# dayae1204/WeCLIP-ViT-CoMer

Measured on AMD Instinct MI355X. Metric: images/sec (train fwd+bwd) ViT-B/16 512x512 VOC, higher is better.
Workload: dtype f16 MFMA operands / f32 accumulate, f32 residual+softmax+LN, PAR f32 arithmetic on 16-bit fixed-point affinities (precision=fast); 1 GPU; WeCLIP VOC full train step (the reference's model: frozen CLIP ViT-B/16 + adapters + decoder + GradCAM/affinity/PAR pseudo-labels), batch 16/GPU at 512x512, K=2 classes/image (BASELINE configs[2] without the ViT-CoMer inserts, for which the reference has no code); global_batch=16, parallelism=dp1

## Files before the change

include/weclip_hip.h:

```cpp
#ifndef WECLIP_HIP_H
#define WECLIP_HIP_H
#include <stdint.h>
#ifdef __cplusplus
extern "C" {
#endif

int wc_version(void);
const char* wc_last_error(void);
int wc_device_count(void);
int wc_device_arch(int dev, char* buf, int buflen);

void wc_prof_enable(int stride);
void wc_prof_tag(const char* tag);
int wc_prof_report(char* buf, int cap);

int wc_par_affinity(const float* img, float* aff, int B, int H, int W,
                    const int* h_dilations, int n_dil, void* stream);
int wc_par_iterate(const float* aff, const float* masks_in, float* masks_out, int B, int C,
                   int H, int W, const int* h_dilations, int n_dil, void* stream);
int wc_par_forward(const float* img, const float* masks, float* out, float* tmp, float* aff_ws,
                   int B, int C, int H, int W, const int* h_dilations, int n_dil, int num_iter,
                   int group, void* stream);
int wc_par_forward_h(const float* img, const float* masks, float* out, float* tmp, float* aff_ws,
                   int B, int C, int H, int W, const int* h_dilations, int n_dil, int num_iter,
// ... 35 lines not shown
int wc_gemm_f16_grouped(const void* A0, const void* A1, const void* A2, const void* W0, const void* W1,
                        const void* W2, int nseg, int M, int N, int K, long lda, long ldw, int batch,
                        long sA, long sW, long sC, const float* bias, const float* resid, long ldr, long sR,
                        float* C32, void* C16, void* C16lo, long ldc, int act, int round16, float scale,
                        int scale_cols, float* P32, const float* aux, const int* rowmap, int rpg,
                        long ldaux, const void* auxh, const float* cscale, long sCS, int zdiv, long sA2, long sW2,
                        long sC2, long sB2, long sX2, void* stream);

int wc_gemm_row_supported(int M, int N, int K);
int wc_gemm_row_f16(const void* A, long lda, const void* W, long ldw, int M, int N, int K, const float* bias,
                    const float* cscale, int act, const float* aux, const void* auxh, long ldaux, const float* resid, long ldr,
                    float* C32, void* C16, float* P32, long ldc, long ldc16, const float* ln_g0, const float* ln_b0, void* ln_o0,
                    const float* ln_g1, const float* ln_b1, void* ln_o1, float eps, void* stream);

int wc_gemm_row_f16_grouped(const void* A, long lda, const void* W, long ldw, int M, int N, int K, const float* bias, int act,
                            const void* auxh, long ldaux, float* C32, void* C16, long ldc, long ldc16, int groups, long gA,
                            long gW, long gB, long gC, long gX, void* stream);

int wc_gemm_plan(int M, int N, int K, int nseg, int batch);
int wc_gemm_log_report(char* buf, int cap);
int wc_sum_slices(const float* part, float* out, int nslices, long n, float alpha, void* stream);

int wc_sum_slices_wb(const float* part, float* out_w, float* out_b, int nslices, int rows, int cols,
                     float alpha, void* stream);
int wc_sum_slices_wb_grouped(const float* part, float* out_w, float* out_b, int nslices, int rows, int cols,
                             float alpha, int groups, long gW, long gB, void* stream);
int wc_sum_slices_wb_multi(const int64_t* jobs, int count, void* stream);

int wc_gemm_km_f16(const void* dY, long lda, const void* X, long ldx, const void* zeros, int M, int N, int K,
                   int x_rpg, int x_gs, int x_off, int mslice, int bias, float* part, void* stream);
int wc_gemm_km_f16_grouped(const void* dY, long lda, const void* X, long ldx, const void* zeros, int M, int N, int K,
                           int x_rpg, int x_gs, int x_off, int mslice, int bias, float* part, int groups, long gA,
                           long gX, void* stream);
int wc_split_f16(const float* x, void* hi, void* lo, long n, void* stream);

int wc_convert_weights(const int64_t* table, int count, int blocks_per_tensor, void* stream);

int wc_adamw_multi(const int64_t* table, int count, double lr, double beta1, double beta2, double eps,
                   double weight_decay, double bias_correction1, double bias_correction2, int blocks_per_tensor,
                   void* stream);

int wc_layernorm(const float* x, long ldx, const float* w, const float* b, float eps, float* y32,
                 void* y16, void* y16lo, long rows, int D, void* stream);

int wc_attn_fwd(const void* qkv, void* out, float* out32, float* lse, int B, int L, int H, int DH,
                void* stream);
int wc_attn_mean(const void* qkv, const float* lse, float* mean, int B, int L, int H, int DH,
                 void* stream);

int wc_patchify(const float* img, void* hi, void* lo, int B, int H, int W, int P, void* stream);
int wc_cls_rows(float* x, const float* cls, const float* pos0, int B, int L, int E, void* stream);

int wc_cam_head(const float* x2, const float* lnw, const float* lnb, const float* proj,
                const float* text, const int* text_idx, const int* n_text, const int* pair_img,
                const int* pair_cls, float logit_scale, float* partial, float* probs, float* df,
                int B, int P, int L, int E, int Ed, int Tmax, void* stream);
int wc_lnpost_bwd(const float* df, const float* x2, const float* lnw, float gs, const int* pair_img,
                  float* d32, void* dhi, void* dlo, int P, int L, int E, void* stream);
int wc_ln2_bwd_add(const float* da2, const float* dx2, const float* x1, const float* lnw, float gs,
                   const int* pair_img, void* g16, int P, int L, int E, void* stream);
int wc_attn_bwd_colsum(const void* qkv, const void* dO, const float* o32, const float* lse,
                       const int* pair_img, float* delta, float* u, float* dS0, float* P0, float* c,
                       int P, int L, int H, int DH, void* stream);
int wc_rowvec_matmul(const float* c, const float* W, float* out, float* ws, int P, int N, int E, float scale,
                     void* stream);
int wc_cam_map(const float* a32, const float* w, const int* pair_img, float* cam, int P, int L, int E,
// ... 170 lines not shown
```

weclip-vit-comer_amd/build.py:

```python
import hashlib
import os
import subprocess
import sys
from concurrent.futures import ThreadPoolExecutor

HERE = os.path.dirname(os.path.abspath(__file__))
CSRC = os.path.join(HERE, "csrc")
OBJ = os.path.join(CSRC, "_build")
LIB = os.path.join(HERE, "libweclip_hip.so")
HIPCC = os.environ.get("HIPCC", "/opt/rocm/bin/hipcc")
FLAGS = ["--offload-arch=gfx950", "-O3", "-fPIC", "-std=c++17", "-ffp-contract=off",
         "-Wno-unused-result", "-I", CSRC] + os.environ.get("WECLIP_HIPCC_FLAGS", "").split()


NO_SCRATCH = ("gemm_row.hip",)


def _sources():
    return sorted(f for f in os.listdir(CSRC) if f.endswith(".hip"))


def _stamp(src):
    h = hashlib.sha1()
    h.update(" ".join("<csrc>" if f == CSRC else f for f in FLAGS).encode())
    for f in [src] + sorted(f for f in os.listdir(CSRC) if f.endswith(".h")):
        with open(os.path.join(CSRC, f), "rb") as fh:
            h.update(fh.read())
    return h.hexdigest()


def source_hash():
    h = hashlib.sha1()
    h.update(" ".join("<csrc>" if f == CSRC else f for f in FLAGS).encode())
    for f in sorted(f for f in os.listdir(CSRC) if f.endswith((".hip", ".h"))):
        with open(os.path.join(CSRC, f), "rb") as fh:
            h.update(f.encode())
            h.update(fh.read())
    return h.hexdigest()[:16]


def _compile(src):
    obj = os.path.join(OBJ, src[:-4] + ".o")
    stamp_file = obj + ".stamp"
    stamp = _stamp(src)
    if os.path.exists(obj) and os.path.exists(stamp_file) and open(stamp_file).read() == stamp:
        return obj, False
    cmd = [HIPCC] + FLAGS + ["-c", os.path.join(CSRC, src), "-o", obj]
    if src in NO_SCRATCH:
# ... 38 lines not shown
```

weclip-vit-comer_amd/comer_engine.py:

```python
import ctypes

import torch

from . import _lib as L
from . import config, ops
from .grad_sink import GradSink, handback, slices
from .ops import F16, F32, Split

GS = 4096.0
INV = 1.0 / GS


_WGRAD_WGS = 256


def _shape_array(shapes):
    return L.int_array([v for hw in shapes for v in hw])


class ComerEngine:
    def __init__(self, net):
        self.net = net
        self.wc = ops.WeightCache()
        self._ref = {}
        self.adapters = None
        self.row_gemm = True

    def params(self):
        net = self.net
        out = []
        for m, c in zip(net.mrfp, net.cti):
            out += [m.fc1.weight, m.fc1.bias, m.fc2.weight, m.fc2.bias, m.dw3.weight, m.dw3.bias, m.dw5.weight, m.dw5.bias]
            out += [c.nv_q.weight, c.nv_q.bias, c.nv_f.weight, c.nv_f.bias, c.gamma, c.nc_q.weight, c.nc_q.bias,
                    c.nc_f.weight, c.nc_f.bias, c.ffn_norm.weight, c.ffn_norm.bias,
                    c.ffn[0].weight, c.ffn[0].bias, c.ffn[2].weight, c.ffn[2].bias]
            for a in (c.to_v, c.to_c):
                out += [a.sampling_offsets.weight, a.sampling_offsets.bias, a.attention_weights.weight, a.attention_weights.bias,
                        a.value_proj.weight, a.value_proj.bias, a.output_proj.weight, a.output_proj.bias]
        out += [net.fuse.weight, net.fuse.bias]
        for a in (self.adapters or []):
            out += [a.proj.weight, a.proj.bias, a.proj_2.weight, a.proj_2.bias]
        return out

    def _mats(self):
        f = lambda t: t.detach() if (t.dtype == F32 and t.is_contiguous()) else t.detach().float().contiguous()
        out = []
        for i, (m, c) in enumerate(zip(self.net.mrfp, self.net.cti)):
            out += [(f"m{i}.fc1", f(m.fc1.weight)), (f"m{i}.fc2", f(m.fc2.weight)), (f"f{i}.0", f(c.ffn[0].weight)),
                    (f"f{i}.2", f(c.ffn[2].weight))]
            for tag, a in (("v", c.to_v), ("c", c.to_c)):
                out += [(f"{tag}{i}.vp", f(a.value_proj.weight)), (f"{tag}{i}.op", f(a.output_proj.weight)),
                        (f"{tag}{i}.ow", [f(a.sampling_offsets.weight), f(a.attention_weights.weight)])]
        out.append(("fuse", f(self.net.fuse.weight).flatten(1)))
# ... 264 lines not shown
                dvs[i] = self._ln_bwd(sink, dq1, s["v"], t.nv_q, dv1)
            df1 = torch.empty(Mc, C, device=dev, dtype=F16)
            self._mm(dval1_16, WT(f"v{i}.vp"), Mc, C, C, out16=df1)
            self._wgrad(sink, dval1_16, s["f1"], Mc, C, C, t.to_v.value_proj)
            if t.nc_q.eps == t.nv_f.eps and C <= 256:
                dc1, dc1_16 = self._ln_bwd2(sink, dq2, t.nc_q, df1, t.nv_f, s["c1"], dc2)
            else:
                dc1 = self._ln_bwd(sink, dq2, s["c1"], t.nc_q, dc2)
                dc1, dc1_16 = self._ln_bwd(sink, df1, s["c1"], t.nv_f, dc1, want16=True)
            dx2 = torch.empty(Mc, hid, device=dev, dtype=F16)
            self._mm(dc1_16, WT(f"m{i}.fc2"), Mc, hid, C, out16=dx2, act=7, aux=s["x2"], ldaux=hid, rpg=1)
            self._wgrad(sink, dc1_16, s["g16"], Mc, C, hid, m.fc2)
            dx1_16 = torch.empty(Mc, hid, device=dev, dtype=F16)
            dw3, db3, dw5, db5 = (sink.dest(q) for q in (m.dw3.weight, m.dw3.bias, m.dw5.weight, m.dw5.bias))
            npart = ctypes.c_long(0)
            lib.wc_mrfp_dwconv_parts(hs3, len(shapes), B, hid, ctypes.byref(npart))
            part = torch.empty(npart.value * hid * 26, device=dev, dtype=F32)
            lib.wc_mrfp_dwconv_bwd(L.ptr(dx2), 1, L.ptr(s["x1"]), L.ptr(self._b(m.dw3.weight).view(-1), F32),
                                   L.ptr(self._b(m.dw5.weight).view(-1), F32), None, L.ptr(dx1_16), L.ptr(dw3), L.ptr(db3), L.ptr(dw5),
                                   L.ptr(db5), L.ptr(part), INV, hs3, len(shapes), B, hid, L.stream())
            dc = torch.empty(Mc, C, device=dev, dtype=F32)
            self._mm(dx1_16, WT(f"m{i}.fc1"), Mc, C, hid, out32=dc, resid=dc1)
            self._wgrad(sink, dx1_16, s["c16"], Mc, hid, C, m.fc1)
            dc3 = dc
        return dc3, dvs

    def _ow_grads(self, sink, dow16, q16, M, n, ld, att):
        K = att.d_model
        outs = [(sink.dest(lin.weight), sink.dest(lin.bias)) for lin in (att.sampling_offsets, att.attention_weights)]
        sink.wgrad(dow16, q16, M, n, K, INV, outs, ns=slices(M, ops.wgrad_tiles(n, K), _WGRAD_WGS), lda=ld)

    def run_backward(self, ctx, dy):
        self._gamma_jobs = []
        with GradSink(self.net.direct_grads) as sink:
            dc0, dvs = self._backward(ctx, dy, sink)
        for t, G, gsum in self._gamma_jobs:
            op = t.to_v.output_proj
            dW, db, dg = (sink.dest(q) for q in (op.weight, op.bias, t.gamma))
            L.lib().wc_cti_gate_grads(L.ptr(G, F32), L.ptr(gsum, F32), L.ptr(self._b(t.gamma), F32), L.ptr(self._b(op.weight), F32),
                                      L.ptr(self._b(op.bias), F32), L.ptr(dW, F32), L.ptr(db, F32), L.ptr(dg, F32), G.shape[0], G.shape[1],
                                      L.stream())
        self._gamma_jobs = None
        B, S, C = ctx["B"], ctx["S"], ctx["C"]
        return (dc0 * INV).view(B, S, C), [d * INV if d is not None else None for d in dvs], sink.grads


class ComerFunction(torch.autograd.Function):

    @staticmethod
    def forward(ctx, engine, shapes, hw, c0, m0, m1, m2, m3, *params):
        y, c = engine.forward(c0, shapes, hw, [m0, m1, m2, m3])
        ctx.engine, ctx.c, ctx.map_shapes = engine, c, [m.shape for m in (m0, m1, m2, m3)]
        return y

    @staticmethod
    def backward(ctx, dy):
        eng = ctx.engine
        dc0, dvs, grads = eng.run_backward(ctx.c, dy.contiguous())
        ctx.c = None
        return (None, None, None, dc0) + tuple(d.view(s) for d, s in zip(dvs, ctx.map_shapes)) + handback(eng.params(), grads)


class ComerTokensFunction(torch.autograd.Function):

    @staticmethod
    def forward(ctx, engine, shapes, hw, Lq, c0, x0, x1, x2, x3, *params):
        y, c = engine.forward(c0, shapes, hw, None, x16=[x0, x1, x2, x3], Lq=Lq)
# ... 10 lines not shown
```

weclip-vit-comer_amd/csrc/gemm_km.hip:

```cpp
#include "gemm_common.h"
#include <cstring>
#include <stdlib.h>

struct KmArgs {
    const __half* A;
    const __half* X;
    const __half* zeros;
    int M, N, K;
    long lda, ldx;
    int x_rpg, x_gs, x_off;
    int mslice;
    int bias;
    int bias_edge;
    int gx;
    int tiles, ns, units;
    int xcd;
    long gA, gX, gP;
    GemmArgs e;
};

typedef short s16x4 __attribute__((__vector_size__(4 * sizeof(short))));
typedef short s16x8 __attribute__((__vector_size__(8 * sizeof(short))));

template <int NST, int HV>
__global__ __launch_bounds__(256 * HV, (HV == 1 && NST <= 5) ? 2 : 1) void gemm_km_kernel(KmArgs g) {
    extern __shared__ __attribute__((aligned(16))) char smem[];
    constexpr int ST = 32 * HV;
    constexpr int TILE = ST * 256;
    constexpr int NT_ = 256 * HV;
    const int tid = threadIdx.x, lane = tid & 63, wave = tid >> 6;
    const int half = HV == 2 ? wave >> 2 : 0, w4 = wave & 3;
    const int wr = w4 >> 1, wc = w4 & 1;
    int unit, tile;
    if (g.xcd) {
        const int chunk = blockIdx.x / (8 * g.tiles), within = blockIdx.x - chunk * (8 * g.tiles);
        unit = chunk * 8 + (within & 7);
        tile = within >> 3;
    } else {
        unit = blockIdx.x / g.tiles;
        tile = blockIdx.x - unit * g.tiles;
    }
    const int grp = unit / g.ns;
    const int z = unit - grp * g.ns;
    const int ty = tile / g.gx, tx = tile - ty * g.gx;
    const int n0 = ty * 128, k0 = tx * 128;
    const __half* Ag = g.A + (long)grp * g.gA;
    const __half* Xg = g.X + (long)grp * g.gX;
    const int mbeg = z * g.mslice;
    const int mend = (mbeg + g.mslice < g.M) ? mbeg + g.mslice : g.M;
    const int nt = (mend - mbeg + ST - 1) / ST;

    int rowi[2], acol[2], xcol[2], xg[2], xr[2];
    unsigned offA[2], offX[2];
    bool aok[2], xok[2];
#pragma unroll
    for (int i = 0; i < 2; ++i) {
        const int q = i * NT_ + tid;
        const int row = q >> 4, pc = q & 15;
        const int lc = pc ^ (((row & 3) << 2) | ((row >> 2) & 3));
        rowi[i] = row;
        acol[i] = n0 + lc * 8;
        xcol[i] = k0 + lc * 8;
        aok[i] = acol[i] + 8 <= g.lda && acol[i] < g.N;
        xok[i] = xcol[i] + 8 <= g.ldx && xcol[i] < g.K;
        const int m = mbeg + row;
        xg[i] = m / g.x_rpg;
        xr[i] = m - xg[i] * g.x_rpg;
        offA[i] = (unsigned)(((long)m * g.lda + (aok[i] ? acol[i] : 0)) * 2);
        offX[i] = (unsigned)((((long)xg[i] * g.x_gs + xr[i] + g.x_off) * g.ldx + (xok[i] ? xcol[i] : 0)) * 2);
    }
    const unsigned dA = (unsigned)(ST * g.lda * 2), dX = (unsigned)(ST * g.ldx * 2);
    const unsigned dXg = (unsigned)(((long)g.x_gs - g.x_rpg) * g.ldx * 2);
    typedef __attribute__((address_space(3))) void* lds_ptr;
    typedef const __attribute__((address_space(1))) void* gbl_ptr;
// ... 132 lines not shown
#pragma unroll
                for (int r = 0; r < 16; ++r) acc[i][j][r] += ex[((i * 2 + j) * 16 + r) * 64];
#pragma unroll
            for (int r = 0; r < 16; ++r) bacc[i][r] += ex[((4 + i) * 16 + r) * 64];
        }
    }
    if (edge_bias) {
        if ((lane & 31) == 0) {
            float* pb = g.e.C32 + (long)z * g.e.sC + (long)grp * g.gP + g.K;
#pragma unroll
            for (int mi = 0; mi < 2; ++mi)
#pragma unroll
                for (int r = 0; r < 16; ++r) {
                    const int row = n0 + wr * 64 + mi * 32 + (r & 3) + 8 * (r >> 2) + 4 * (lane >> 5);
                    if (row < g.N) pb[(long)row * g.e.ldc] = bacc[mi][r];
                }
        }
    } else if (own_bias) {
        const int ni = kb >> 5, cl = kb & 31;
        if ((lane & 31) == cl) {
#pragma unroll
            for (int mi = 0; mi < 2; ++mi)
#pragma unroll
                for (int r = 0; r < 16; ++r) {
                    if (ni == 0) acc[mi][0][r] = bacc[mi][r];
                    else acc[mi][1][r] = bacc[mi][r];
                }
        }
    }
    const float bv[2] = {0.f, 0.f}, sc[2] = {1.f, 1.f};
    gemm_epilogue<0>(g.e, acc, n0, k0, wr, wc, lane, z, smem + w4 * 8192, bv, sc, (long)z * g.e.sC + (long)grp * g.gP);
}

extern "C" int wc_gemm_km_f16_grouped(const void* dY, long lda, const void* X, long ldx, const void* zeros, int M, int N,
                                      int K, int x_rpg, int x_gs, int x_off, int mslice, int bias, float* part, int groups,
                                      long gA, long gX, void* stream) {
    WC_CHECK_ARG(dY && X && zeros && part && M > 0 && N > 0 && K > 0, "wc_gemm_km_f16: bad argument");
    WC_CHECK_ARG(groups >= 1 && groups <= 65535 && gA % 8 == 0 && gX % 8 == 0, "wc_gemm_km_f16_grouped: bad group strides");
    WC_CHECK_ARG(lda % 8 == 0 && ldx % 8 == 0 && lda >= N && ldx >= K && ((uintptr_t)dY | (uintptr_t)X | (uintptr_t)zeros) % 16 == 0,
                 "wc_gemm_km_f16: operand rows must be 16-byte aligned (lda, ldx %% 8 == 0)");
    WC_CHECK_ARG(mslice > 0 && mslice % 64 == 0, "wc_gemm_km_f16: mslice must be a positive multiple of 64");
    WC_CHECK_ARG(x_rpg >= 1 && x_gs >= 0 && x_off >= 0, "wc_gemm_km_f16: bad row map");
    {
        const long xrows = (long)((M - 1) / x_rpg) * x_gs + (x_rpg - 1 < M - 1 ? x_rpg - 1 : M - 1) + x_off + 1;
        WC_CHECK_ARG((long)M * lda * 2 < (1L << 32) && xrows * ldx * 2 < (1L << 32), "wc_gemm_km_f16: operands of 4 GiB and more are not supported");
    }
    const int ns = wc_cdiv(M, mslice);
    WC_CHECK_ARG(ns <= 65535, "wc_gemm_km_f16: too many slices");
    KmArgs g = {};
    g.A = (const __half*)dY; g.X = (const __half*)X; g.zeros = (const __half*)zeros;
    g.M = M; g.N = N; g.K = K; g.lda = lda; g.ldx = ldx;
    g.x_rpg = x_rpg; g.x_gs = x_gs; g.x_off = x_off; g.mslice = mslice; g.bias = bias ? 1 : 0;
    const int K1 = K + g.bias;
    g.bias_edge = (g.bias && K % 128 == 0) ? 1 : 0;
    g.gx = g.bias_edge ? K / 128 : wc_cdiv(K1, 128);
    GemmArgs& e = g.e;
    e.nseg = 1; e.M = N; e.N = K1; e.sC = (long)N * K1; e.C32 = part; e.ldc = K1;
    e.scale = 1.f; e.rpg = 1; e.zdiv = 1; e.gx = g.gx; e.gy = wc_cdiv(N, 128);
    g.gA = gA; g.gX = gX; g.gP = (long)ns * N * K1;
    g.tiles = g.gx * wc_cdiv(N, 128); g.ns = ns; g.units = groups * ns;
    g.xcd = g.units % 8 == 0 ? 1 : 0;
    WC_CHECK_ARG((long)g.tiles * g.units < (1L << 31), "wc_gemm_km_f16: grid too large");
    dim3 grid((unsigned)(g.tiles * g.units));
    const int pr = wc_prof_begin(stream);
    const int sl = shape_log_begin(stream);
    static bool lds_attr_set = false;
    if (!lds_attr_set) {
        WC_CHECK_ARG(hipFuncSetAttribute((const void*)gemm_km_kernel<4, 2>, hipFuncAttributeMaxDynamicSharedMemorySize, 4 * 128 * 256) == hipSuccess &&
                         hipFuncSetAttribute((const void*)gemm_km_kernel<5, 1>, hipFuncAttributeMaxDynamicSharedMemorySize, 5 * 64 * 256) == hipSuccess,
                     "wc_gemm_km_f16: cannot reserve 128 KiB of LDS");
        lds_attr_set = true;
    }
    if ((long)g.tiles * g.units <= gemm_cu_count() && mslice >= 128)
        hipLaunchKernelGGL((gemm_km_kernel<4, 2>), grid, dim3(512), 4 * 128 * 256, (hipStream_t)stream, g);
    else
        hipLaunchKernelGGL((gemm_km_kernel<5, 1>), grid, dim3(256), 5 * 64 * 256, (hipStream_t)stream, g);
    shape_log_end(sl, "km", M, N, K1, 1, groups, ns, 0, stream);
    wc_prof_end(pr, "gemm_km_kernel", 2.0 * M * N * K1 * groups, stream);
    WC_LAUNCH_CHECK("gemm_km_kernel");
    return WC_OK;
}

extern "C" int wc_gemm_km_f16(const void* dY, long lda, const void* X, long ldx, const void* zeros, int M, int N, int K,
                              int x_rpg, int x_gs, int x_off, int mslice, int bias, float* part, void* stream) {
    return wc_gemm_km_f16_grouped(dY, lda, X, ldx, zeros, M, N, K, x_rpg, x_gs, x_off, mslice, bias, part, 1, 0, 0, stream);
}

__global__ __launch_bounds__(256) void sum_slices_kernel(const float* __restrict__ part, float* __restrict__ out,
                                                          int nslices, long n, float alpha) {
    const long i = (long)blockIdx.x * 256 + threadIdx.x;
    if (i >= n) return;
    float s0 = 0.f, s1 = 0.f, s2 = 0.f, s3 = 0.f;
    int k = 0;
    for (; k + 4 <= nslices; k += 4) {
        s0 += part[(long)k * n + i];
        s1 += part[(long)(k + 1) * n + i];
        s2 += part[(long)(k + 2) * n + i];
        s3 += part[(long)(k + 3) * n + i];
    }
    for (; k < nslices; ++k) s0 += part[(long)k * n + i];
    out[i] = ((s0 + s1) + (s2 + s3)) * alpha;
}

__global__ __launch_bounds__(256) void sum_slices_wb_kernel(const float* __restrict__ part, float* __restrict__ out_w,
                                                             float* __restrict__ out_b, int nslices, int rows, int cols,
                                                             float alpha, long gW, long gB) {
    const long n = (long)rows * (cols + 1);
    part += (long)blockIdx.y * nslices * n;
    out_w += (long)blockIdx.y * gW;
    out_b += (long)blockIdx.y * gB;
    const long i = (long)blockIdx.x * 256 + threadIdx.x;
    if (i >= n) return;
    float s0 = 0.f, s1 = 0.f, s2 = 0.f, s3 = 0.f;
    int k = 0;
    for (; k + 4 <= nslices; k += 4) {
        s0 += part[(long)k * n + i];
        s1 += part[(long)(k + 1) * n + i];
        s2 += part[(long)(k + 2) * n + i];
// ... 123 lines not shown
```

weclip-vit-comer_amd/grad_sink.py:

```python
import ctypes
import struct

import torch

from . import _lib as L
from . import ops
from .ops import F32


def slices(M, tiles, budget):
    ns = 1
    while ns * 2 * tiles <= budget and M // (ns * 2) >= 256:
        ns *= 2
    return ns


def handback(params, grads):
    out = []
    for p in params:
        g = grads.get(id(p))
        if g is not None and p.grad is not None and g.data_ptr() == p.grad.data_ptr():
            g = None
        out.append(g.reshape(p.shape) if g is not None else None)
    return tuple(out)


class GradSink:

    def __init__(self, bucket=None):
        self.bucket = bucket
        self.grads = {}
        self._jobs = []

    def __enter__(self):
        return self

    def __exit__(self, exc, *_):
        if exc is None:
            self.flush()

    def direct(self, p):
        g = p.grad
        if self.bucket is None or g is None or not g.is_contiguous() or g.dtype != F32 or g.data_ptr() % 16:
            return None
        lo, hi = self.bucket
        return g if lo <= g.data_ptr() and g.data_ptr() + 4 * g.numel() <= hi else None

    def dest(self, p):
        g = self.direct(p)
        if g is None:
            g = torch.empty(p.shape, device=p.device, dtype=F32)
        self.grads[id(p)] = g
        return g

    def put(self, params, grads):
        for p, g in zip(params, grads):
            self.grads[id(p)] = g

    def ln_dest(self, weight, bias):
        gw, gb = self.direct(weight), self.direct(bias)
        if gw is None or gb is None or gb.data_ptr() != gw.data_ptr() + 4 * gw.numel():
            return None
        return torch.as_strided(gw, (2, gw.numel()), (gw.numel(), 1))

    def wgrad(self, dy16, x16, M, N, K, alpha, outs, *, ns, groups=1, sw=0, sb=0, **kw):
        if sum(db.numel() for _, db in outs) != N:
            raise ValueError("GradSink.wgrad: the destinations do not cover the N gradient rows")
        part, ns = ops.wgrad_partials(dy16, x16, M, N, K, slices=ns, bias=True, groups=groups, **kw)
        abits = struct.unpack("<I", struct.pack("<f", alpha))[0]
        stride = N * (K + 1)
        r0 = 0
        for dw, db in outs:
            rows = db.numel()
            for g in range(groups):
                self._jobs.append(((part, dw, db), [part.data_ptr() + 4 * (g * ns * stride + r0 * (K + 1)),
                                                    dw.data_ptr() + 4 * g * sw, db.data_ptr() + 4 * g * sb,
                                                    ns, rows, K, abits, stride]))
            r0 += rows

    def flush(self):
        jobs, self._jobs = self._jobs, []
        if jobs:
            flat = [v for _, fields in jobs for v in fields]
            L.lib().wc_sum_slices_wb_multi((ctypes.c_int64 * len(flat))(*flat), len(jobs), L.stream())
```

weclip-vit-comer_amd/head_engine.py:

```python
import os

import torch

from . import config, ops
from .clip import vit_engine as VE
from .grad_sink import GradSink, handback, slices
from .ops import F16, F32, Split

GRAD_SCALE = 4096.0
_WGRAD_WGS = 512


def _f(p):
    return p.detach().float().contiguous()


def _uniform_stride(ts):
    p = [t.data_ptr() for t in ts]
    if len(p) < 2:
        return None
    d = p[1] - p[0]
    es = ts[0].element_size()
    if d <= 0 or d % (8 * es) or any(p[i + 1] - p[i] != d for i in range(len(p) - 1)) or \
            any(t.shape != ts[0].shape for t in ts):
        return None
    return d // es


class HeadEngine:
    def __init__(self, fuse, dec, attn_pred=True):
        self.fuse, self.dec = fuse, dec
        self.attn_pred = bool(attn_pred)
        self.E = dec.linear_pred.weight.shape[1]
        self.nc = dec.linear_pred.weight.shape[0]
        self.index = fuse.indexes
        self.direct_grads = None
        self.fwd_stream = None
        self.row_gemm = True
        self.wcache = ops.WeightCache()

    def params(self):
        return list(self.fuse.parameters()) + list(self.dec.parameters())

    def dec_params(self):
        return list(self.dec.parameters())

    def _weight_matrices(self):
        out = []
        for l, mlp in enumerate(self.fuse.linears_modulelist):
            out.append((f"ad{l}.proj", mlp.proj.weight.detach()))
            out.append((f"ad{l}.proj_2", mlp.proj_2.weight.detach()))
        out.append(("fuse", self.fuse.linear_fuse.weight.detach().flatten(1)))
        out.append(("pred", self.dec.linear_pred.weight.detach().flatten(1)))
        for i, blk in enumerate(self.dec.transformer.resblocks):
            out += [(f"b{i}.in", blk.attn.in_proj_weight.detach()), (f"b{i}.out", blk.attn.out_proj.weight.detach()),
                    (f"b{i}.fc", blk.mlp.c_fc.weight.detach()), (f"b{i}.pj", blk.mlp.c_proj.weight.detach())]
        return [(n, t if t.dtype == F32 and t.is_contiguous() else t.float().contiguous()) for n, t in out]

    def forward(self, xs, B, Lq, h, w, drop_scale=None, F_rows=None):
        ex = config.exact()
        E, hw, M = self.E, h * w, B * h * w
        n = self.index
# ... 71 lines not shown
        x3 = blocks[-1]["x2h"]
        seg_rows = torch.empty(M, self.nc, device=dev, dtype=F32)
        ops.gemm(x3, wc.w("pred"), M, self.nc, E,
                 bias=_f(self.dec.linear_pred.bias), out32=seg_rows)
        seg = seg_rows.view(B, h, w, self.nc).permute(0, 3, 1, 2).contiguous()
        if not self.attn_pred:
            ctx["ap"] = None
            return seg, None, ctx
        ap = torch.empty(B, hw, hw, device=dev, dtype=F32)
        ops.gemm(Fh, Fh, hw, hw, E, out32=ap, act=3, batch=B, sA=hw * E, sW=hw * E, sC=hw * hw)
        ctx["ap"] = ap
        return seg, ap, ctx

    def _block_fwd(self, pk, x, B, Lq):
        M, E, H, DH = B * Lq, pk.E, pk.H, pk.DH
        dev = x.device
        ex = pk.exact
        _, a = ops.layernorm(x, pk.ln1_w, pk.ln1_b, with_lo=ex)
        qkv = torch.empty(M, 3 * E, device=dev, dtype=F16)
        ops.gemm(a, pk.in_w, M, 3 * E, E, bias=pk.in_b, out16=qkv, scale=ops.q_scale(DH), scale_cols=E)
        o16, lse, _, o32 = ops.attention(qkv, B, Lq, H, DH, want_mean=False, want_o32=True)
        x1 = torch.empty(M, E, device=dev, dtype=F32)
        ops.gemm(o16, pk.out_w, M, E, E, bias=pk.out_b, resid=x, out32=x1, round16=True)
        _, a2 = ops.layernorm(x1, pk.ln2_w, pk.ln2_b, with_lo=ex)
        z = Split(torch.empty(M, 4 * E, device=dev, dtype=F16), torch.empty(M, 4 * E, device=dev, dtype=F16) if ex else None)
        u32 = torch.empty(M, 4 * E, device=dev, dtype=F32)
        ops.gemm(a2, pk.fc_w, M, 4 * E, E, bias=pk.fc_b, out16=z.hi, out16lo=z.lo, act=1, pre32=u32)
        x2 = torch.empty(M, E, device=dev, dtype=F32)
        x2h = Split(torch.empty(M, E, device=dev, dtype=F16), torch.empty(M, E, device=dev, dtype=F16) if ex else None)
        ops.gemm(z, pk.pj_w, M, E, 4 * E, bias=pk.pj_b, resid=x1, out32=x2, out16=x2h.hi, out16lo=x2h.lo)
        return x2, dict(x=x, a=a, qkv=qkv, o16=o16, o32=o32, lse=lse, x1=x1, a2=a2, u32=u32, z=z, x2h=x2h)

    def backward(self, ctx, dseg, dap):
        with GradSink(self.direct_grads) as sink:
            dF = self._backward_impl(ctx, dseg, dap, sink)
        return sink.grads, dF

    def _backward_impl(self, ctx, dseg, dap, sink):
        B, h, w, ex = ctx["B"], ctx["h"], ctx["w"], ctx["ex"]
        E, hw, M, nc, n = self.E, h * w, B * h * w, self.nc, self.index
        dev = ctx["F32"].device
        GS, inv = GRAD_SCALE, 1.0 / GRAD_SCALE
        wg = lambda dy16, x16, N_, K_, pw, pb, **kw: self._wgrad(sink, dy16, x16, M, N_, K_, inv, pw, pb, **kw)
        x3h = ctx["blocks"][-1]["x2h"]
        pred = self.dec.linear_pred
        if dseg is not None:
            wpT, ldT = self.wcache.wT("pred")
            d = torch.zeros(M, ldT, device=dev, dtype=F32)
            d[:, :nc] = dseg.permute(0, 2, 3, 1).reshape(M, nc)
            _, dS = ops.colscale_split(d, None, M, alpha=GS, want32=False, with_lo=ex)
            dx = torch.empty(M, E, device=dev, dtype=F32)
            ops.gemm(dS, wpT, M, E, ldT, out32=dx)
            wg(dS.hi, x3h.hi, nc, E, pred.weight, pred.bias, lda=ldT)
        else:
            dx = torch.zeros(M, E, device=dev, dtype=F32)
            sink.dest(pred.weight).zero_()
            sink.dest(pred.bias).zero_()
        for i in reversed(range(len(ctx["blocks"]))):
            dx = self._block_bwd(ctx["blocks"][i], dx, B, hw, sink, inv)
        if dap is not None:
            S = ops.sigmoid_gram_bwd(dap.contiguous(), ctx["ap"], scale=GS, with_lo=ex)
            hwp = S.hi.shape[-1]
            FT, Kp = ops.transpose_f16(ctx["F32"], hw, E, batch=B, sSrc=hw * E, oR=hwp)
            dF = torch.empty(M, E, device=dev, dtype=F32)
            ops.gemm(S, FT, hw, E, hwp, lda=hwp, ldw=Kp, out32=dF, resid=dx, batch=B, sA=hw * hwp, sW=hwp, sC=hw * E)
        else:
            dF = dx
# ... 149 lines not shown
```

weclip-vit-comer_amd/ops.py:

```python
import math

import torch

from . import _lib as L

F16 = torch.float16
F32 = torch.float32
LOG2E = 1.4426950408889634


class KernelTimer:

    active = False

    @staticmethod
    def enable(stride=1):
        L.lib().cdll.wc_prof_enable(int(stride))
        KernelTimer.active = bool(stride)
        if not stride:
            L.lib().cdll.wc_prof_tag(None)

    @staticmethod
    def tag(name):
        if KernelTimer.active:
            L.lib().cdll.wc_prof_tag(name)

    @staticmethod
    def summary():
        import ctypes
        buf = ctypes.create_string_buffer(1 << 16)
        L.lib().cdll.wc_prof_report(buf, len(buf))
        out = {}
# ... 171 lines not shown
    return d


def transpose_f16(src, R, C, *, ld=None, batch=1, sSrc=0, with_lo=False, scale=1.0, oR=None, ones_row=False):
    ld = C if ld is None else ld
    oR = R if oR is None else oR
    K = (batch - 1) * oR + R
    Kp = (batch * oR + 63) // 64 * 64
    dev = src.device
    alloc = torch.zeros if Kp != K else torch.empty
    rows = C + 1 if ones_row else C
    hi = alloc(rows, Kp, device=dev, dtype=F16)
    lo = alloc(rows, Kp, device=dev, dtype=F16) if with_lo else None
    if ones_row:
        if oR != R:
            raise RuntimeError("ones_row needs densely packed batches")
        hi[C, :K] = 1.0
        if lo is not None:
            lo[C].zero_()
    f32 = src.dtype == F32
    L.lib().wc_transpose_f16(L.ptr(src, F32 if f32 else F16, "src"), 1 if f32 else 0, ld, sSrc, L.ptr(hi), L.ptr(lo),
                             Kp, oR, batch, R, C, float(scale), L.stream())
    return Split(hi, lo), Kp


_ZEROS = {}


def wgrad_tiles(N, K, bias=True):
    kt = K // 128 if (bias and K % 128 == 0) else (K + (1 if bias else 0) + 127) // 128
    return ((N + 127) // 128) * kt


def wgrad_partials(dy16, x16, M, N, K, *, lda=None, ldx=None, slices=1, bias=True, xmap=None, groups=1, gA=0, gX=0):
    L.require_gpu()
    lda = N if lda is None else lda
    ldx = K if ldx is None else ldx
    dev = dy16.device
    z = _ZEROS.get(dev)
    if z is None:
        z = _ZEROS[dev] = torch.zeros(64, device=dev, dtype=F16)
    mslice = (-(-M // slices) + 63) // 64 * 64
    ns = -(-M // mslice)
    K1 = K + (1 if bias else 0)
    part = torch.empty((ns, N, K1) if groups == 1 else (groups, ns, N, K1), device=dev, dtype=F32)
    rpg, gs, off = xmap if xmap is not None else (max(M, 64), 0, 0)
    L.lib().wc_gemm_km_f16_grouped(L.ptr(dy16, F16, "dY"), lda, L.ptr(x16, F16, "X"), ldx, L.ptr(z), M, N, K, rpg, gs, off,
                                   mslice, 1 if bias else 0, L.ptr(part), groups, gA, gX, L.stream())
    return part, ns


def colsum(src, R, C, *, ld=None, alpha=1.0, round16=False, out=None):
    ld = C if ld is None else ld
    dev = src.device
    part = torch.empty(((R + 255) // 256) * C, device=dev, dtype=F32)
    out = torch.empty(C, device=dev, dtype=F32) if out is None else out
    f32 = src.dtype == F32
    L.lib().wc_colsum(L.ptr(src, F32 if f32 else F16, "src"), 1 if f32 else 0, ld, L.ptr(part), L.ptr(out, F32), R, C,
                      float(alpha), 1 if round16 else 0, L.stream())
    return out


def layernorm_bwd(dy, x, w, *, add=None, want32=True, want16=False, out_scale=1.0, alpha=1.0, eps=1e-5, dgb=None):
    rows, D = x.shape
    dev = x.device
    dx32 = torch.empty(rows, D, device=dev, dtype=F32) if want32 else None
    dx16 = torch.empty(rows, D, device=dev, dtype=F16) if want16 else None
    part = torch.empty(((rows + 15) // 16) * 2 * D, device=dev, dtype=F32)
    if dgb is None:
        dgb = torch.empty(2, D, device=dev, dtype=F32)
    fn = L.lib().wc_layernorm_bwd_h if dy.dtype == F16 else L.lib().wc_layernorm_bwd
    fn(L.ptr(dy, dy.dtype, "dy"), L.ptr(x, F32, "x"), L.ptr(w, F32, "w"), L.ptr(add, F32, "add"), eps,
       L.ptr(dx32), L.ptr(dx16), float(out_scale), L.ptr(part), L.ptr(dgb), float(alpha), rows, D, L.stream())
    return dx32, dx16, dgb


def layernorm_bwd2(dya, wa, dyb, wb, x, *, add=None, want32=True, want16=False, out_scale=1.0, alpha=1.0, eps=1e-5, dgba=None, dgbb=None):
    rows, D = x.shape
    dev = x.device
    dx32 = torch.empty(rows, D, device=dev, dtype=F32) if want32 else None
    dx16 = torch.empty(rows, D, device=dev, dtype=F16) if want16 else None
    part = torch.empty(min((rows + 15) // 16, 2048) * 4 * D, device=dev, dtype=F32)
# ... 82 lines not shown
```

Baseline: 1272 images/sec.

## Batch deferred weight-gradient GEMMs into grouped multi-job kernel launches

Weight-gradient GEMMs in the backward passes of the comer and head engines are now queued and flushed together at the end of the pass. A new multi-job kernel packs up to 32 jobs into one grid, sorted by slice length and split by the HV form, with a per-block job lookup. This cuts launch overhead and lets small wgrad GEMMs fill the GPU together. In exchange, the queued tensors stay alive longer, the wgrads no longer overlap with the dgrad chain, and each block pays a small job-lookup cost.

```diff
diff --git a/include/weclip_hip.h b/include/weclip_hip.h
--- a/include/weclip_hip.h
+++ b/include/weclip_hip.h
@@ -91,6 +91,10 @@
 int wc_gemm_km_f16_grouped(const void* dY, long lda, const void* X, long ldx, const void* zeros, int M, int N, int K,
                            int x_rpg, int x_gs, int x_off, int mslice, int bias, float* part, int groups, long gA,
                            long gX, void* stream);
+int wc_gemm_km_f16_multi(const int64_t* jobs, int count, const void* zeros, void* stream);
+int wc_gemm_km_multi_plan(const int64_t* jobs, int count, int cus, int* launch, int* first, int* pos, int* grids,
+                          int* forms, int max_launches, int* nlaunches);
+int wc_gemm_km_multi_locate(const int64_t* jobs, int count, int cus, int l, int wg, int* out);
 int wc_split_f16(const float* x, void* hi, void* lo, long n, void* stream);
 
 int wc_convert_weights(const int64_t* table, int count, int blocks_per_tensor, void* stream);
diff --git a/weclip-vit-comer_amd/build.py b/weclip-vit-comer_amd/build.py
--- a/weclip-vit-comer_amd/build.py
+++ b/weclip-vit-comer_amd/build.py
@@ -13,7 +13,7 @@
          "-Wno-unused-result", "-I", CSRC] + os.environ.get("WECLIP_HIPCC_FLAGS", "").split()
 
 
-NO_SCRATCH = ("gemm_row.hip",)
+NO_SCRATCH = ("gemm_row.hip", "gemm_km.hip")
 
 
 def _sources():
diff --git a/weclip-vit-comer_amd/comer_engine.py b/weclip-vit-comer_amd/comer_engine.py
--- a/weclip-vit-comer_amd/comer_engine.py
+++ b/weclip-vit-comer_amd/comer_engine.py
@@ -19,6 +19,8 @@
 
 
 class ComerEngine:
+    defer_wgrads = True
+
     def __init__(self, net):
         self.net = net
         self.wc = ops.WeightCache()
@@ -349,7 +351,7 @@
 
     def run_backward(self, ctx, dy):
         self._gamma_jobs = []
-        with GradSink(self.net.direct_grads) as sink:
+        with GradSink(self.net.direct_grads, defer=self.defer_wgrads) as sink:
             dc0, dvs = self._backward(ctx, dy, sink)
         for t, G, gsum in self._gamma_jobs:
             op = t.to_v.output_proj
diff --git a/weclip-vit-comer_amd/csrc/gemm_km.hip b/weclip-vit-comer_amd/csrc/gemm_km.hip
--- a/weclip-vit-comer_amd/csrc/gemm_km.hip
+++ b/weclip-vit-comer_amd/csrc/gemm_km.hip
@@ -1,6 +1,7 @@
 #include "gemm_common.h"
 #include <cstring>
 #include <stdlib.h>
+#include <vector>
 
 struct KmArgs {
     const __half* A;
@@ -19,11 +20,22 @@
     GemmArgs e;
 };
 
+__host__ __device__ __forceinline__ void km_unit_tile(int bid, int tiles, int xcd, int& unit, int& tile) {
+    if (xcd) {
+        const int chunk = bid / (8 * tiles), within = bid - chunk * (8 * tiles);
+        unit = chunk * 8 + (within & 7);
+        tile = within >> 3;
+    } else {
+        unit = bid / tiles;
+        tile = bid - unit * tiles;
+    }
+}
+
 typedef short s16x4 __attribute__((__vector_size__(4 * sizeof(short))));
 typedef short s16x8 __attribute__((__vector_size__(8 * sizeof(short))));
 
 template <int NST, int HV>
-__global__ __launch_bounds__(256 * HV, (HV == 1 && NST <= 5) ? 2 : 1) void gemm_km_kernel(KmArgs g) {
+__device__ __forceinline__ void gemm_km_body(const KmArgs& g, const int bid) {
     extern __shared__ __attribute__((aligned(16))) char smem[];
     constexpr int ST = 32 * HV;
     constexpr int TILE = ST * 256;
@@ -32,14 +44,7 @@
     const int half = HV == 2 ? wave >> 2 : 0, w4 = wave & 3;
     const int wr = w4 >> 1, wc = w4 & 1;
     int unit, tile;
-    if (g.xcd) {
-        const int chunk = blockIdx.x / (8 * g.tiles), within = blockIdx.x - chunk * (8 * g.tiles);
-        unit = chunk * 8 + (within & 7);
-        tile = within >> 3;
-    } else {
-        unit = blockIdx.x / g.tiles;
-        tile = blockIdx.x - unit * g.tiles;
-    }
+    km_unit_tile(bid, g.tiles, g.xcd, unit, tile);
     const int grp = unit / g.ns;
     const int z = unit - grp * g.ns;
     const int ty = tile / g.gx, tx = tile - ty * g.gx;
@@ -238,58 +243,244 @@
     gemm_epilogue<0>(g.e, acc, n0, k0, wr, wc, lane, z, smem + w4 * 8192, bv, sc, (long)z * g.e.sC + (long)grp * g.gP);
 }
 
+template <int NST, int HV>
+__global__ __launch_bounds__(256 * HV, (HV == 1 && NST <= 5) ? 2 : 1) void gemm_km_kernel(KmArgs g) {
+    gemm_km_body<NST, HV>(g, blockIdx.x);
+}
+
+__host__ __device__ __forceinline__ void km_fill(KmArgs& g, const __half* A, const __half* X, const __half* zeros, float* part, int M,
+                                                 int N, int K, long lda, long ldx, int x_rpg, int x_gs, int x_off, int mslice,
+                                                 int bias, int ns, int units, long gA, long gX) {
+    g.A = A; g.X = X; g.zeros = zeros;
+    g.M = M; g.N = N; g.K = K; g.lda = lda; g.ldx = ldx;
+    g.x_rpg = x_rpg; g.x_gs = x_gs; g.x_off = x_off; g.mslice = mslice; g.bias = bias ? 1 : 0;
+    const int K1 = K + g.bias, gy = (N + 127) / 128;
+    g.bias_edge = (g.bias && K % 128 == 0) ? 1 : 0;
+    g.gx = g.bias_edge ? K / 128 : (K1 + 127) / 128;
+    GemmArgs& e = g.e;
+    e.nseg = 1; e.M = N; e.N = K1; e.sC = (long)N * K1; e.C32 = part; e.ldc = K1;
+    e.scale = 1.f; e.rpg = 1; e.zdiv = 1; e.gx = g.gx; e.gy = gy;
+    g.gA = gA; g.gX = gX; g.gP = (long)ns * N * K1;
+    g.tiles = g.gx * gy; g.ns = ns; g.units = units;
+    g.xcd = units % 8 == 0 ? 1 : 0;
+}
+
+struct KmJob {
+    const void* dY; const void* X; float* part;
+    int M, N, K; long lda, ldx; int x_rpg, x_gs, x_off, mslice, bias, groups; long gA, gX;
+    int ns, wgs, hv;
+};
+
+static int km_check(KmJob& j, int cus) {
+    WC_CHECK_ARG(j.dY && j.X && j.part && j.M > 0 && j.N > 0 && j.K > 0, "wc_gemm_km_f16: bad argument");
+    WC_CHECK_ARG(j.groups >= 1 && j.groups <= 65535 && j.gA % 8 == 0 && j.gX % 8 == 0, "wc_gemm_km_f16_grouped: bad group strides");
+    WC_CHECK_ARG(j.lda % 8 == 0 && j.ldx % 8 == 0 && j.lda >= j.N && j.ldx >= j.K && ((uintptr_t)j.dY | (uintptr_t)j.X) % 16 == 0,
+                 "wc_gemm_km_f16: operand rows must be 16-byte aligned (lda, ldx %% 8 == 0)");
+    WC_CHECK_ARG(j.mslice > 0 && j.mslice % 64 == 0, "wc_gemm_km_f16: mslice must be a positive multiple of 64");
+    WC_CHECK_ARG(j.x_rpg >= 1 && j.x_gs >= 0 && j.x_off >= 0, "wc_gemm_km_f16: bad row map");
+    {
+        const int M = j.M;
+        const long xrows = (long)((M - 1) / j.x_rpg) * j.x_gs + (j.x_rpg - 1 < M - 1 ? j.x_rpg - 1 : M - 1) + j.x_off + 1;
+        WC_CHECK_ARG((long)M * j.lda * 2 < (1L << 32) && xrows * j.ldx * 2 < (1L << 32), "wc_gemm_km_f16: operands of 4 GiB and more are not supported");
+    }
+    j.ns = wc_cdiv(j.M, j.mslice);
+    WC_CHECK_ARG(j.ns <= 65535, "wc_gemm_km_f16: too many slices");
+    KmArgs g = {};
+    km_fill(g, nullptr, nullptr, nullptr, nullptr, j.M, j.N, j.K, j.lda, j.ldx, j.x_rpg, j.x_gs, j.x_off, j.mslice, j.bias, j.ns,
+            j.groups * j.ns, j.gA, j.gX);
+    WC_CHECK_ARG((long)g.tiles * g.units < (1L << 31), "wc_gemm_km_f16: grid too large");
+    j.wgs = g.tiles * g.units;
+    j.hv = (j.wgs <= (cus > 0 ? cus : gemm_cu_count()) && j.mslice >= 128) ? 2 : 1;
+    return WC_OK;
+}
+
+static int km_reserve_lds();
+
 extern "C" int wc_gemm_km_f16_grouped(const void* dY, long lda, const void* X, long ldx, const void* zeros, int M, int N,
                                       int K, int x_rpg, int x_gs, int x_off, int mslice, int bias, float* part, int groups,
                                       long gA, long gX, void* stream) {
-    WC_CHECK_ARG(dY && X && zeros && part && M > 0 && N > 0 && K > 0, "wc_gemm_km_f16: bad argument");
-    WC_CHECK_ARG(groups >= 1 && groups <= 65535 && gA % 8 == 0 && gX % 8 == 0, "wc_gemm_km_f16_grouped: bad group strides");
-    WC_CHECK_ARG(lda % 8 == 0 && ldx % 8 == 0 && lda >= N && ldx >= K && ((uintptr_t)dY | (uintptr_t)X | (uintptr_t)zeros) % 16 == 0,
-                 "wc_gemm_km_f16: operand rows must be 16-byte aligned (lda, ldx %% 8 == 0)");
-    WC_CHECK_ARG(mslice > 0 && mslice % 64 == 0, "wc_gemm_km_f16: mslice must be a positive multiple of 64");
-    WC_CHECK_ARG(x_rpg >= 1 && x_gs >= 0 && x_off >= 0, "wc_gemm_km_f16: bad row map");
-    {
-        const long xrows = (long)((M - 1) / x_rpg) * x_gs + (x_rpg - 1 < M - 1 ? x_rpg - 1 : M - 1) + x_off + 1;
-        WC_CHECK_ARG((long)M * lda * 2 < (1L << 32) && xrows * ldx * 2 < (1L << 32), "wc_gemm_km_f16: operands of 4 GiB and more are not supported");
-    }
-    const int ns = wc_cdiv(M, mslice);
-    WC_CHECK_ARG(ns <= 65535, "wc_gemm_km_f16: too many slices");
+    WC_CHECK_ARG(zeros && (uintptr_t)zeros % 16 == 0, "wc_gemm_km_f16: bad argument");
+    KmJob j = {dY, X, part, M, N, K, lda, ldx, x_rpg, x_gs, x_off, mslice, bias, groups, gA, gX, 0, 0, 0};
+    if (const int rc = km_check(j, 0)) return rc;
     KmArgs g = {};
-    g.A = (const __half*)dY; g.X = (const __half*)X; g.zeros = (const __half*)zeros;
-    g.M = M; g.N = N; g.K = K; g.lda = lda; g.ldx = ldx;
-    g.x_rpg = x_rpg; g.x_gs = x_gs; g.x_off = x_off; g.mslice = mslice; g.bias = bias ? 1 : 0;
-    const int K1 = K + g.bias;
-    g.bias_edge = (g.bias && K % 128 == 0) ? 1 : 0;
-    g.gx = g.bias_edge ? K / 128 : wc_cdiv(K1, 128);
-    GemmArgs& e = g.e;
-    e.nseg = 1; e.M = N; e.N = K1; e.sC = (long)N * K1; e.C32 = part; e.ldc = K1;
-    e.scale = 1.f; e.rpg = 1; e.zdiv = 1; e.gx = g.gx; e.gy = wc_cdiv(N, 128);
-    g.gA = gA; g.gX = gX; g.gP = (long)ns * N * K1;
-    g.tiles = g.gx * wc_cdiv(N, 128); g.ns = ns; g.units = groups * ns;
-    g.xcd = g.units % 8 == 0 ? 1 : 0;
-    WC_CHECK_ARG((long)g.tiles * g.units < (1L << 31), "wc_gemm_km_f16: grid too large");
-    dim3 grid((unsigned)(g.tiles * g.units));
+    km_fill(g, (const __half*)dY, (const __half*)X, (const __half*)zeros, part, M, N, K, lda, ldx, x_rpg, x_gs, x_off, mslice, bias,
+            j.ns, groups * j.ns, gA, gX);
+    dim3 grid((unsigned)j.wgs);
     const int pr = wc_prof_begin(stream);
     const int sl = shape_log_begin(stream);
+    if (const int rc = km_reserve_lds()) return rc;
+    if (j.hv == 2)
+        hipLaunchKernelGGL((gemm_km_kernel<4, 2>), grid, dim3(512), 4 * 128 * 256, (hipStream_t)stream, g);
+    else
+        hipLaunchKernelGGL((gemm_km_kernel<5, 1>), grid, dim3(256), 5 * 64 * 256, (hipStream_t)stream, g);
+    shape_log_end(sl, "km", M, N, g.e.N, 1, groups, j.ns, 0, stream);
+    wc_prof_end(pr, "gemm_km_kernel", 2.0 * M * N * g.e.N * groups, stream);
+    WC_LAUNCH_CHECK("gemm_km_kernel");
+    return WC_OK;
+}
+
+extern "C" int wc_gemm_km_f16(const void* dY, long lda, const void* X, long ldx, const void* zeros, int M, int N, int K,
+                              int x_rpg, int x_gs, int x_off, int mslice, int bias, float* part, void* stream) {
+    return wc_gemm_km_f16_grouped(dY, lda, X, ldx, zeros, M, N, K, x_rpg, x_gs, x_off, mslice, bias, part, 1, 0, 0, stream);
+}
+
+#define KMJ_MAX 32
+struct KmJobs {
+    const __half* zeros;
+    int first[KMJ_MAX];
+    const __half* A[KMJ_MAX];
+    const __half* X[KMJ_MAX];
+    float* P[KMJ_MAX];
+    long gA[KMJ_MAX], gX[KMJ_MAX];
+    int M[KMJ_MAX], N[KMJ_MAX], K[KMJ_MAX], lda[KMJ_MAX], ldx[KMJ_MAX], x_rpg[KMJ_MAX], x_gs[KMJ_MAX], x_off[KMJ_MAX];
+    int mslice[KMJ_MAX], bias[KMJ_MAX], ns[KMJ_MAX], units[KMJ_MAX];
+};
+static_assert(sizeof(KmJobs) <= 3072, "KmJobs must stay well under the 4 KiB kernel-argument limit");
+
+__host__ __device__ __forceinline__ int km_find_job(const int* first, int bid) {
+    int q = 0;
+#pragma unroll
+    for (int i = 1; i < KMJ_MAX; ++i) q += bid >= first[i] ? 1 : 0;
+    return q;
+}
+
+template <int NST, int HV>
+__global__ __launch_bounds__(256 * HV, (HV == 1 && NST <= 5) ? 2 : 1) void gemm_km_multi_kernel(KmJobs j) {
+    const int q = km_find_job(j.first, blockIdx.x);
+    KmArgs g = {};
+    km_fill(g, j.A[q], j.X[q], j.zeros, j.P[q], j.M[q], j.N[q], j.K[q], j.lda[q], j.ldx[q], j.x_rpg[q], j.x_gs[q], j.x_off[q],
+            j.mslice[q], j.bias[q], j.ns[q], j.units[q], j.gA[q], j.gX[q]);
+    const int bid = blockIdx.x - j.first[q];
+    if (bid >= g.tiles * g.units) return;
+    gemm_km_body<NST, HV>(g, bid);
+}
+
+static int km_reserve_lds() {
     static bool lds_attr_set = false;
     if (!lds_attr_set) {
         WC_CHECK_ARG(hipFuncSetAttribute((const void*)gemm_km_kernel<4, 2>, hipFuncAttributeMaxDynamicSharedMemorySize, 4 * 128 * 256) == hipSuccess &&
-                         hipFuncSetAttribute((const void*)gemm_km_kernel<5, 1>, hipFuncAttributeMaxDynamicSharedMemorySize, 5 * 64 * 256) == hipSuccess,
+                         hipFuncSetAttribute((const void*)gemm_km_kernel<5, 1>, hipFuncAttributeMaxDynamicSharedMemorySize, 5 * 64 * 256) == hipSuccess &&
+                         hipFuncSetAttribute((const void*)gemm_km_multi_kernel<4, 2>, hipFuncAttributeMaxDynamicSharedMemorySize, 4 * 128 * 256) == hipSuccess &&
+                         hipFuncSetAttribute((const void*)gemm_km_multi_kernel<5, 1>, hipFuncAttributeMaxDynamicSharedMemorySize, 5 * 64 * 256) == hipSuccess,
                      "wc_gemm_km_f16: cannot reserve 128 KiB of LDS");
         lds_attr_set = true;
     }
-    if ((long)g.tiles * g.units <= gemm_cu_count() && mslice >= 128)
-        hipLaunchKernelGGL((gemm_km_kernel<4, 2>), grid, dim3(512), 4 * 128 * 256, (hipStream_t)stream, g);
-    else
-        hipLaunchKernelGGL((gemm_km_kernel<5, 1>), grid, dim3(256), 5 * 64 * 256, (hipStream_t)stream, g);
-    shape_log_end(sl, "km", M, N, K1, 1, groups, ns, 0, stream);
-    wc_prof_end(pr, "gemm_km_kernel", 2.0 * M * N * K1 * groups, stream);
-    WC_LAUNCH_CHECK("gemm_km_kernel");
-    return WC_OK;
-}
-
-extern "C" int wc_gemm_km_f16(const void* dY, long lda, const void* X, long ldx, const void* zeros, int M, int N, int K,
-                              int x_rpg, int x_gs, int x_off, int mslice, int bias, float* part, void* stream) {
-    return wc_gemm_km_f16_grouped(dY, lda, X, ldx, zeros, M, N, K, x_rpg, x_gs, x_off, mslice, bias, part, 1, 0, 0, stream);
+    return WC_OK;
+}
+
+struct KmLaunch { int hv, n, grid; int job[KMJ_MAX], first[KMJ_MAX]; };
+#define KM_JOB_FIELDS 16
+static int km_plan(const int64_t* jobs, int count, int cus, KmJob* js, KmLaunch* ls, int max_launches, int* nl) {
+    int* order = (int*)alloca(sizeof(int) * count);
+    for (int i = 0; i < count; ++i) {
+        const int64_t* e = jobs + (long)i * KM_JOB_FIELDS;
+        for (int k = 3; k < 14; ++k) WC_CHECK_ARG(e[k] >= 0 && e[k] < (1L << 31), "wc_gemm_km_f16_multi: job field out of range");
+        js[i] = KmJob{reinterpret_cast<const void*>(e[0]), reinterpret_cast<const void*>(e[1]), reinterpret_cast<float*>(e[2]),
+                      (int)e[3], (int)e[4], (int)e[5], (long)e[6], (long)e[7], (int)e[8], (int)e[9], (int)e[10], (int)e[11],
+                      (int)e[12], (int)e[13], (long)e[14], (long)e[15], 0, 0, 0};
+        if (const int rc = km_check(js[i], cus)) return rc;
+        const int len = js[i].M < js[i].mslice ? js[i].M : js[i].mslice;
+        int p = i;
+        for (; p > 0; --p) {
+            const KmJob& o = js[order[p - 1]];
+            if ((o.M < o.mslice ? o.M : o.mslice) >= len) break;
+            order[p] = order[p - 1];
+        }
+        order[p] = i;
+    }
+    *nl = 0;
+    for (int hv = 1; hv <= 2; ++hv) {
+        KmLaunch* cur = nullptr;
+        for (int p = 0; p < count; ++p) {
+            const KmJob& j = js[order[p]];
+            if (j.hv != hv) continue;
+            if (!cur || cur->n == KMJ_MAX || (long)cur->grid + j.wgs + 8 >= (1L << 31)) {
+                WC_CHECK_ARG(*nl < max_launches, "wc_gemm_km_f16_multi: too many launches");
+                cur = ls + (*nl)++;
+                cur->hv = hv; cur->n = 0; cur->grid = 0;
+            }
+            cur->job[cur->n] = order[p];
+            cur->first[cur->n] = cur->grid;
+            cur->n += 1;
+            cur->grid += (j.wgs + 7) / 8 * 8;
+        }
+    }
+    return WC_OK;
+}
+
+static void km_table(const KmLaunch& l, const KmJob* js, const void* zeros, KmJobs& t) {
+    t.zeros = (const __half*)zeros;
+    for (int q = 0; q < KMJ_MAX; ++q) {
+        const KmJob& j = js[l.job[q < l.n ? q : 0]];
+        t.first[q] = q < l.n ? l.first[q] : 0x7fffffff;
+        t.A[q] = (const __half*)j.dY; t.X[q] = (const __half*)j.X; t.P[q] = j.part;
+        t.gA[q] = j.gA; t.gX[q] = j.gX;
+        t.M[q] = j.M; t.N[q] = j.N; t.K[q] = j.K; t.lda[q] = (int)j.lda; t.ldx[q] = (int)j.ldx;
+        t.x_rpg[q] = j.x_rpg; t.x_gs[q] = j.x_gs; t.x_off[q] = j.x_off; t.mslice[q] = j.mslice; t.bias[q] = j.bias;
+        t.ns[q] = j.ns; t.units[q] = j.groups * j.ns;
+    }
+}
+
+extern "C" int wc_gemm_km_f16_multi(const int64_t* jobs, int count, const void* zeros, void* stream) {
+    WC_CHECK_ARG(jobs && count > 0 && count <= 4096 && zeros && (uintptr_t)zeros % 16 == 0, "wc_gemm_km_f16_multi: bad argument");
+    std::vector<KmJob> js(count);
+    std::vector<KmLaunch> ls(2 * (count / KMJ_MAX + 1));
+    int nl = 0;
+    if (const int rc = km_plan(jobs, count, 0, js.data(), ls.data(), (int)ls.size(), &nl)) return rc;
+    if (const int rc = km_reserve_lds()) return rc;
+    for (int i = 0; i < nl; ++i) {
+        KmJobs t;
+        km_table(ls[i], js.data(), zeros, t);
+        double flops = 0;
+        for (int q = 0; q < ls[i].n; ++q) {
+            const KmJob& j = js[ls[i].job[q]];
+            flops += 2.0 * j.M * j.N * (j.K + (j.bias ? 1 : 0)) * j.groups;
+        }
+        const int pr = wc_prof_begin(stream);
+        if (ls[i].hv == 2)
+            hipLaunchKernelGGL((gemm_km_multi_kernel<4, 2>), dim3((unsigned)ls[i].grid), dim3(512), 4 * 128 * 256, (hipStream_t)stream, t);
+        else
+            hipLaunchKernelGGL((gemm_km_multi_kernel<5, 1>), dim3((unsigned)ls[i].grid), dim3(256), 5 * 64 * 256, (hipStream_t)stream, t);
+        wc_prof_end(pr, "gemm_km_multi_kernel", flops, stream);
+        WC_LAUNCH_CHECK("gemm_km_multi_kernel");
+    }
+    return WC_OK;
+}
+
+extern "C" int wc_gemm_km_multi_plan(const int64_t* jobs, int count, int cus, int* launch, int* first, int* pos, int* grids,
+                                     int* forms, int max_launches, int* nlaunches) {
+    WC_CHECK_ARG(jobs && count > 0 && count <= 4096 && launch && first && pos && grids && forms && nlaunches && max_launches > 0,
+                 "wc_gemm_km_multi_plan: bad argument");
+    std::vector<KmJob> js(count);
+    std::vector<KmLaunch> ls(max_launches);
+    if (const int rc = km_plan(jobs, count, cus, js.data(), ls.data(), max_launches, nlaunches)) return rc;
+    for (int l = 0; l < *nlaunches; ++l) {
+        grids[l] = ls[l].grid; forms[l] = ls[l].hv;
+        for (int q = 0; q < ls[l].n; ++q) { launch[ls[l].job[q]] = l; first[ls[l].job[q]] = ls[l].first[q]; pos[ls[l].job[q]] = q; }
+    }
+    return WC_OK;
+}
+
+extern "C" int wc_gemm_km_multi_locate(const int64_t* jobs, int count, int cus, int l, int wg, int* out) {
+    WC_CHECK_ARG(jobs && count > 0 && count <= 4096 && out && l >= 0 && wg >= 0, "wc_gemm_km_multi_locate: bad argument");
+    std::vector<KmJob> js(count);
+    std::vector<KmLaunch> ls(2 * (count / KMJ_MAX + 1));
+    int nl = 0;
+    if (const int rc = km_plan(jobs, count, cus, js.data(), ls.data(), (int)ls.size(), &nl)) return rc;
+    WC_CHECK_ARG(l < nl && wg < ls[l].grid, "wc_gemm_km_multi_locate: no such workgroup");
+    KmJobs t;
+    km_table(ls[l], js.data(), nullptr, t);
+    const int q = km_find_job(t.first, wg);
+    KmArgs g = {};
+    km_fill(g, t.A[q], t.X[q], t.zeros, t.P[q], t.M[q], t.N[q], t.K[q], t.lda[q], t.ldx[q], t.x_rpg[q], t.x_gs[q], t.x_off[q],
+            t.mslice[q], t.bias[q], t.ns[q], t.units[q], t.gA[q], t.gX[q]);
+    const int bid = wg - t.first[q];
+    out[0] = -1; out[1] = out[2] = 0;
+    if (bid < g.tiles * g.units) {
+        out[0] = ls[l].job[q];
+        km_unit_tile(bid, g.tiles, g.xcd, out[1], out[2]);
+    }
+    return WC_OK;
 }
 
 __global__ __launch_bounds__(256) void sum_slices_kernel(const float* __restrict__ part, float* __restrict__ out,
diff --git a/weclip-vit-comer_amd/grad_sink.py b/weclip-vit-comer_amd/grad_sink.py
--- a/weclip-vit-comer_amd/grad_sink.py
+++ b/weclip-vit-comer_amd/grad_sink.py
@@ -27,8 +27,10 @@
 
 class GradSink:
 
-    def __init__(self, bucket=None):
+    def __init__(self, bucket=None, defer=True):
         self.bucket = bucket
+        self.defer = defer
+        self._gemms = []
         self.grads = {}
         self._jobs = []
 
@@ -66,6 +68,8 @@
     def wgrad(self, dy16, x16, M, N, K, alpha, outs, *, ns, groups=1, sw=0, sb=0, **kw):
         if sum(db.numel() for _, db in outs) != N:
             raise ValueError("GradSink.wgrad: the destinations do not cover the N gradient rows")
+        if self.defer:
+            kw["queue"] = self._gemms
         part, ns = ops.wgrad_partials(dy16, x16, M, N, K, slices=ns, bias=True, groups=groups, **kw)
         abits = struct.unpack("<I", struct.pack("<f", alpha))[0]
         stride = N * (K + 1)
@@ -79,6 +83,7 @@
             r0 += rows
 
     def flush(self):
+        ops.wgrad_launch(self._gemms)
         jobs, self._jobs = self._jobs, []
         if jobs:
             flat = [v for _, fields in jobs for v in fields]
diff --git a/weclip-vit-comer_amd/head_engine.py b/weclip-vit-comer_amd/head_engine.py
--- a/weclip-vit-comer_amd/head_engine.py
+++ b/weclip-vit-comer_amd/head_engine.py
@@ -28,6 +28,8 @@
 
 
 class HeadEngine:
+    defer_wgrads = True
+
     def __init__(self, fuse, dec, attn_pred=True):
         self.fuse, self.dec = fuse, dec
         self.attn_pred = bool(attn_pred)
@@ -165,7 +167,7 @@
         return x2, dict(x=x, a=a, qkv=qkv, o16=o16, o32=o32, lse=lse, x1=x1, a2=a2, u32=u32, z=z, x2h=x2h)
 
     def backward(self, ctx, dseg, dap):
-        with GradSink(self.direct_grads) as sink:
+        with GradSink(self.direct_grads, defer=self.defer_wgrads) as sink:
             dF = self._backward_impl(ctx, dseg, dap, sink)
         return sink.grads, dF
 
diff --git a/weclip-vit-comer_amd/ops.py b/weclip-vit-comer_amd/ops.py
--- a/weclip-vit-comer_amd/ops.py
+++ b/weclip-vit-comer_amd/ops.py
@@ -1,3 +1,4 @@
+import ctypes
 import math
 
 import torch
@@ -235,22 +236,38 @@
     return ((N + 127) // 128) * kt
 
 
-def wgrad_partials(dy16, x16, M, N, K, *, lda=None, ldx=None, slices=1, bias=True, xmap=None, groups=1, gA=0, gX=0):
+def wgrad_partials(dy16, x16, M, N, K, *, lda=None, ldx=None, slices=1, bias=True, xmap=None, groups=1, gA=0, gX=0, queue=None):
     L.require_gpu()
     lda = N if lda is None else lda
     ldx = K if ldx is None else ldx
     dev = dy16.device
-    z = _ZEROS.get(dev)
-    if z is None:
-        z = _ZEROS[dev] = torch.zeros(64, device=dev, dtype=F16)
     mslice = (-(-M // slices) + 63) // 64 * 64
     ns = -(-M // mslice)
     K1 = K + (1 if bias else 0)
     part = torch.empty((ns, N, K1) if groups == 1 else (groups, ns, N, K1), device=dev, dtype=F32)
     rpg, gs, off = xmap if xmap is not None else (max(M, 64), 0, 0)
-    L.lib().wc_gemm_km_f16_grouped(L.ptr(dy16, F16, "dY"), lda, L.ptr(x16, F16, "X"), ldx, L.ptr(z), M, N, K, rpg, gs, off,
+    if queue is not None:
+        queue.append(((dy16, x16, part), [L.ptr(dy16, F16, "dY").value, L.ptr(x16, F16, "X").value, part.data_ptr(), M, N, K, lda,
+                                          ldx, rpg, gs, off, mslice, 1 if bias else 0, groups, gA, gX]))
+        return part, ns
+    L.lib().wc_gemm_km_f16_grouped(L.ptr(dy16, F16, "dY"), lda, L.ptr(x16, F16, "X"), ldx, L.ptr(_zeros(dev)), M, N, K, rpg, gs, off,
                                    mslice, 1 if bias else 0, L.ptr(part), groups, gA, gX, L.stream())
     return part, ns
+
+
+def _zeros(dev):
+    z = _ZEROS.get(dev)
+    if z is None:
+        z = _ZEROS[dev] = torch.zeros(64, device=dev, dtype=F16)
+    return z
+
+
+def wgrad_launch(queue):
+    jobs = list(queue)
+    del queue[:]
+    if jobs:
+        flat = [v for _, fields in jobs for v in fields]
+        L.lib().wc_gemm_km_f16_multi((ctypes.c_int64 * len(flat))(*flat), len(jobs), L.ptr(_zeros(jobs[0][0][0].device)), L.stream())
 
 
 def colsum(src, R, C, *, ld=None, alpha=1.0, round16=False, out=None):
```

Measured after the change: 1293 images/sec (median of 6 runs). 1.6% higher.
